# vmonardo/pnp-svrg

Measured on AMD Instinct MI355X. Metric: PnP-SVRG inner-iters/sec, 256x256 CSMRI+DnCNN, higher is better.
Workload: dtype f32; 1 GPU; pnp_svrg (true SVRG direction, T2=10, mb=1000) on 256x256 CSMRI, 20% Bernoulli mask, DnCNN-17 prox (reference DnCNN_noise15 weights); batch_per_gpu=120, problems_total=120, parallelism=replicas x1 (no data-path collective)

## Files before the change

### include/pnp_hip.h

```cpp
#ifndef PNP_HIP_H
#define PNP_HIP_H
#include <stddef.h>
#include <stdint.h>

#ifdef __cplusplus
extern "C" {
#endif

enum { PNP_F32 = 0, PNP_F64 = 1 };
enum { PNP_OK = 0, PNP_ERR_ARG = 1, PNP_ERR_HIP = 2, PNP_ERR_UNSUPPORTED = 3 };

int pnp_version(void);
const char* pnp_last_error(void);

typedef struct pnp_csmri_plan pnp_csmri_plan;

int pnp_csmri_plan_create(pnp_csmri_plan** plan, int H, int W, int batch, int dtype);
int pnp_csmri_plan_destroy(pnp_csmri_plan* plan);

int pnp_csmri_sel_from_indices(pnp_csmri_plan* plan, const int32_t* idx, int n, uint8_t* selT, void* stream);
int pnp_csmri_pack_mask(pnp_csmri_plan* plan, const uint8_t* selT, uint32_t* bitsT, void* stream);

int pnp_csmri_draw_thresholds(pnp_csmri_plan* plan, const uint32_t* bitsT, int mb, uint64_t seed, uint32_t step0,
                              int nsteps, const uint32_t* step_dev, void* mbd, uint32_t* selbits, void* stream);
// ... 62 lines not shown

int pnp_minmax(const void* z, int n_per_problem, int batch, int dtype, void* out, void* stream);

typedef struct pnp_dncnn_plan pnp_dncnn_plan;
int pnp_dncnn_plan_create(pnp_dncnn_plan** plan, int n_mid, const float* w_first, const float* w_mid,
                          const float* b_mid, const float* w_last, int H, int W, int batch);
int pnp_dncnn_plan_destroy(pnp_dncnn_plan* plan);
int pnp_dncnn_set_affine(pnp_dncnn_plan* plan, const float* b_first, float b_last, float negative_slope);
int pnp_dncnn_set_winograd(pnp_dncnn_plan* plan, int enable);
int pnp_dncnn_forward(pnp_dncnn_plan* plan, const float* x, float* r, void* stream);
int pnp_dncnn_denoise(pnp_dncnn_plan* plan, const void* z_in, void* z_out, int dtype, double sigma_net,
                      const void* xrec, double* sse_out, void* stream);

int pnp_mmo_denoise(pnp_dncnn_plan* plan, const void* z_in, void* z_out, int dtype, const void* xrec,
                    double* sse_out, void* stream);

int pnp_dncnn_profile_begin(pnp_dncnn_plan* plan, int max_calls);
int pnp_dncnn_profile_end(pnp_dncnn_plan* plan, double* avg_ms_per_launch, long* launches);
int pnp_dncnn_debug_clock(pnp_dncnn_plan* plan, int reps, double* cycles, double* ref_ticks, void* stream);
size_t pnp_dncnn_debug_w44_floats(void);
int pnp_dncnn_debug_w44_weights(pnp_dncnn_plan* plan, int layer, float* dst, void* stream);
int pnp_dncnn_debug_mid_layer(pnp_dncnn_plan* plan, int layer, const float* in, float* out, const float* w44_override,
                              int w44_rows, void* stream);

int pnp_counter_add(uint32_t* counter, uint32_t inc, void* stream);
int pnp_log_append(const double* src, int n, double* log, int n_log, const uint32_t* step_dev, void* stream);
int pnp_log_append_inc(const double* src, int n, double* log, int n_log, uint32_t* counter, void* stream);

int pnp_draw_thresholds(int M, int batch, int mb, uint64_t seed, uint32_t step0, int nsteps, const uint32_t* step_dev,
                        void* mbd, void* stream);
int pnp_indicator_from_thresholds(int M, int batch, const void* mbd, uint8_t* sel, void* stream);
int pnp_rows_from_thresholds(int M, int batch, int mb, const void* mbd, int32_t* rows, void* stream);
int pnp_indicator_from_indices(const int32_t* idx, int n, int M, int batch, uint8_t* sel, void* stream);
int pnp_saga_table_update(void* z, const void* g, void* slot, const void* prev, void* sum, double lr, double inv_hist,
                          size_t n, int dtype, void* stream);

int pnp_axpbypcz(double a, const void* x, double b, const void* y, double c, const void* w,
                 void* out, size_t n, int dtype, void* stream);

int pnp_legacy_choice(uint32_t* mt_key, int* mt_pos, const int64_t* pool, int pop, int size, int32_t* work, int64_t* out);

#ifdef __cplusplus
}
#endif
#endif
```

### pnp_svrg_amd/_native.py

```python
import ctypes
import os

_HERE = os.path.dirname(os.path.abspath(__file__))
LIB_PATH = os.environ.get('PNP_HIP_LIB') or os.path.join(_HERE, 'lib', 'libpnp_hip.so')

F32, F64 = 0, 1

_vp = ctypes.c_void_p
_i = ctypes.c_int
_d = ctypes.c_double
_sz = ctypes.c_size_t

SIGNATURES = {
    'pnp_version': (_i, []),
    'pnp_last_error': (ctypes.c_char_p, []),
    'pnp_csmri_plan_create': (_i, [ctypes.POINTER(_vp), _i, _i, _i, _i]),
    'pnp_csmri_plan_destroy': (_i, [_vp]),
    'pnp_csmri_sel_from_indices': (_i, [_vp, _vp, _i, _vp, _vp]),
    'pnp_csmri_pack_mask': (_i, [_vp, _vp, _vp, _vp]),
    'pnp_csmri_draw_thresholds': (_i, [_vp, _vp, _i, ctypes.c_uint64, ctypes.c_uint32, _i, _vp, _vp, _vp, _vp]),
    'pnp_csmri_sel_from_thresholds': (_i, [_vp, _vp, _vp, _vp, _vp]),
    'pnp_csmri_draw_minibatch': (_i, [_vp, _vp, _i, ctypes.c_uint64, ctypes.c_uint32, _vp, _vp, _vp]),
    'pnp_counter_add': (_i, [_vp, ctypes.c_uint32, _vp]),
    'pnp_log_append': (_i, [_vp, _i, _vp, _i, _vp, _vp]),
# ... 12 lines not shown
    'pnp_deblur_forward': (_i, [_vp, _vp, _vp, _vp]),
    'pnp_pr_workspace_elems': (_sz, [_i, _i]),
    'pnp_pr_grad': (_i, [_vp, _vp, _vp, _vp, _i, _i, _i, _i, _d, _vp, _vp, _vp]),
    'pnp_pr_grad_batch': (_i, [_vp, _vp, _vp, _vp, _i, _i, _i, _i, _i, _d, _vp, _vp, _vp]),
    'pnp_pr_spectral_apply': (_i, [_vp, _vp, _vp, _i, _i, _i, _d, _vp, _vp, _vp]),
    'pnp_sigma_est': (_i, [_vp, _i, _i, _i, _i, _vp, _vp]),
    'pnp_prox_tv': (_i, [_vp, _vp, _i, _i, _i, _i, _vp, _d, _d, _vp, _vp, _vp, _vp]),
    'pnp_nlm2d': (_i, [_vp, _vp, _i, _i, _i, _i, _i, _i, _vp, _d, _d, _vp, _d, _vp, _vp, _vp, _vp]),
    'pnp_sse': (_i, [_vp, _vp, _i, _i, _i, _vp, _vp]),
    'pnp_minmax': (_i, [_vp, _i, _i, _i, _vp, _vp]),
    'pnp_dncnn_plan_create': (_i, [ctypes.POINTER(_vp), _i, _vp, _vp, _vp, _vp, _i, _i, _i]),
    'pnp_dncnn_plan_destroy': (_i, [_vp]),
    'pnp_dncnn_set_affine': (_i, [_vp, _vp, ctypes.c_float, ctypes.c_float]),
    'pnp_dncnn_set_winograd': (_i, [_vp, _i]),
    'pnp_dncnn_forward': (_i, [_vp, _vp, _vp, _vp]),
    'pnp_dncnn_denoise': (_i, [_vp, _vp, _vp, _i, _d, _vp, _vp, _vp]),
    'pnp_mmo_denoise': (_i, [_vp, _vp, _vp, _i, _vp, _vp, _vp]),
    'pnp_dncnn_profile_begin': (_i, [_vp, _i]),
    'pnp_dncnn_profile_end': (_i, [_vp, ctypes.POINTER(_d), ctypes.POINTER(ctypes.c_long)]),
    'pnp_dncnn_debug_clock': (_i, [_vp, _i, ctypes.POINTER(_d), ctypes.POINTER(_d), _vp]),
    'pnp_dncnn_debug_w44_floats': (_sz, []),
    'pnp_dncnn_debug_w44_weights': (_i, [_vp, _i, _vp, _vp]),
    'pnp_dncnn_debug_mid_layer': (_i, [_vp, _i, _vp, _vp, _vp, _i, _vp]),
    'pnp_draw_thresholds': (_i, [_i, _i, _i, ctypes.c_uint64, ctypes.c_uint32, _i, _vp, _vp, _vp]),
    'pnp_indicator_from_thresholds': (_i, [_i, _i, _vp, _vp, _vp]),
    'pnp_rows_from_thresholds': (_i, [_i, _i, _i, _vp, _vp, _vp]),
    'pnp_indicator_from_indices': (_i, [_vp, _i, _i, _i, _vp, _vp]),
    'pnp_saga_table_update': (_i, [_vp, _vp, _vp, _vp, _vp, _d, _d, _sz, _i, _vp]),
    'pnp_axpbypcz': (_i, [_d, _vp, _d, _vp, _d, _vp, _vp, _sz, _i, _vp]),
    'pnp_legacy_choice': (_i, [_vp, ctypes.POINTER(ctypes.c_int), _vp, _i, _i, _vp, _vp]),
}

_lib = None


class NativeError(RuntimeError):
    pass


def lib():
    global _lib
    if _lib is None:
        if not os.path.exists(LIB_PATH):
            raise NativeError(
                f'{LIB_PATH} not found: build it with `python -c "import __graft_entry__ as g; g.build()"` '
                '(or `make -C pnp_svrg_amd/csrc`). There is no CPU fallback.')
# ... 18 lines not shown
```

### pnp_svrg_amd/csrc/dncnn.hip

```cpp
#include "common.h"
#include "wino44.h"
#include "wino44b.h"
#include "tilewalk.h"
#include "reduce.h"
#include <vector>
#include <algorithm>
#include <cstdlib>

namespace pnp {

using f32x4 = __attribute__((ext_vector_type(4))) float;

constexpr int C = 64;
constexpr int TR = 8, TC = 32;
constexpr int PR = TR + 2;
constexpr int PC = 40;
constexpr int XOFF = 3;
constexpr int PLANE = PR * PC;
constexpr int HALF_C = 32;
constexpr int HALF_PAYLOAD = HALF_C * PLANE;
constexpr int HALF_LDS = 52 * 256;
constexpr int CHUNKS = HALF_PAYLOAD / 4;
constexpr int KSTEPS_HALF = 9 * (HALF_C / 4);
constexpr int MT = 16;

__device__ __forceinline__ void dma_piece(int pc, const float* __restrict__ in, const float* __restrict__ zeros,
                                          float* ldsbuf, int H, int W, int b, int ty0, int tx0, int half, int lane,
                                          bool valid_tile) {
    const int q = pc * 64 + lane;
    const int cin = q / 100, r = q - cin * 100;
// ... 450 lines not shown
                const T lo = mm[2 * b], hi = mm[2 * b + 1];
                T v = (zin[p] - lo) / (hi - lo);
                v = v * (T)srange + (T)sshift;
                v = v - (T)r[j];
                v = (v - (T)sshift) / (T)srange;
                v = v * (hi - lo) + lo;
                zout[p] = v;
                if (xrec != nullptr) {
                    const double d = (double)xrec[p] - (double)v;
                    err += d * d;
                }
            }
        }
    }
    if (sse_part != nullptr) {
        err = wave_sum(err);
        if ((tid & 63) == 0) red[tid >> 6] = err;
        __syncthreads();
        if (tid == 0)
            sse_part[((size_t)b * gridDim.y + blockIdx.y) * gridDim.x + blockIdx.x] = red[0] + red[1] + red[2] + red[3];
    }
}

__global__ void k_sum_parts(const double* __restrict__ part, int nparts, double* __restrict__ out) {
    double s = 0;
    for (int i = threadIdx.x; i < nparts; i += 64) s += part[(size_t)blockIdx.x * nparts + i];
    s = wave_sum(s);
    if (threadIdx.x == 0) out[blockIdx.x] = s;
}

}

using namespace pnp;

struct pnp_dncnn_plan {
    int n_mid, H, W, batch, num_cu;
    float *w_first, *w_last, *wpack, *upack, *bias;
    float* upack44;
    uint16_t* upack44b;
    float* b_first;
    float b_last, slope;
    int use_wino;
    float *act0, *act1, *zeros;
    double* mm;
    double* sse_part;
    bool profile;
    std::vector<hipEvent_t> ev;
    size_t ev_used;
    double prof_ms;
    long prof_launches;
};

extern "C" int pnp_dncnn_plan_create(pnp_dncnn_plan** out, int n_mid, const float* w_first, const float* w_mid,
                                     const float* b_mid, const float* w_last, int H, int W, int batch) {
    PNP_CHECK_ARG(out && w_first && w_mid && b_mid && w_last, "null argument");
    PNP_CHECK_ARG(n_mid >= 1 && batch >= 1, "n_mid and batch must be >= 1");
    PNP_CHECK_ARG(H % TR == 0 && W % TC == 0 && (H * W) % 256 == 0, "H must be a multiple of 8, W of 32");
    auto* p = new pnp_dncnn_plan{};
    p->n_mid = n_mid; p->H = H; p->W = W; p->batch = batch;
    hipDeviceProp_t prop;
    int dev = 0;
    PNP_CHECK_HIP(hipGetDevice(&dev));
    PNP_CHECK_HIP(hipGetDeviceProperties(&prop, dev));
    p->num_cu = prop.multiProcessorCount;
    std::vector<float> pack((size_t)n_mid * 4 * 2 * KSTEPS_HALF * 64);
// ... 3 lines not shown
                for (int lane = 0; lane < 64; ++lane) {
                    const int half = s / KSTEPS_HALF, rs = s % KSTEPS_HALF, tap = rs / (HALF_C / 4), c4 = rs % (HALF_C / 4);
                    const int cout = 16 * wv + (lane & 15), cin = HALF_C * half + 4 * c4 + (lane >> 4);
                    pack[(((size_t)l * 4 + wv) * 2 * KSTEPS_HALF + s) * 64 + lane] =
                        w_mid[(((size_t)l * C + cout) * C + cin) * 9 + tap];
                }
    std::vector<float> upk((size_t)n_mid * 4 * WINO_U * 64);
    for (int l = 0; l < n_mid; ++l)
        for (int wv = 0; wv < 4; ++wv)
            for (int s = 0; s < WINO_U; ++s)
                for (int lane = 0; lane < 64; ++lane) {
                    const int xi = s % 4, dy = (s / 4) % 3, c4 = (s / 12) % (HALF_C / 4), half = s / (12 * (HALF_C / 4));
                    const int cout = 16 * wv + (lane & 15), cin = HALF_C * half + 4 * c4 + (lane >> 4);
                    const float* g = w_mid + (((size_t)l * C + cout) * C + cin) * 9 + dy * 3;
                    const double g0 = g[0], g1 = g[1], g2 = g[2];
                    const double u = xi == 0 ? g0 : xi == 1 ? 0.5 * (g0 + g1 + g2) : xi == 2 ? 0.5 * (g0 - g1 + g2) : g2;
                    upk[(((size_t)l * 4 + wv) * WINO_U + s) * 64 + lane] = (float)u;
                }
    {
        const char* ev = getenv("PNP_DNCNN_WINOGRAD");
        p->use_wino = ev ? atoi(ev) : 5;
        if (p->use_wino != 6 && p->use_wino != 5 && p->use_wino != 1 && p->use_wino != 0) p->use_wino = 5;
        if (p->use_wino >= 5 && !wino44_supports(H, W)) p->use_wino = 1;
    }
    const size_t act_bytes = (size_t)batch * C * H * W * sizeof(float);
    hipError_t e = hipMalloc(&p->wpack, pack.size() * sizeof(float));
    if (e == hipSuccess) e = hipMemcpy(p->wpack, pack.data(), pack.size() * sizeof(float), hipMemcpyHostToDevice);
    if (e == hipSuccess) e = hipMalloc(&p->upack, upk.size() * sizeof(float));
    if (e == hipSuccess) e = hipMemcpy(p->upack, upk.data(), upk.size() * sizeof(float), hipMemcpyHostToDevice);
    {
        std::vector<float> u44(wino44_weight_floats(n_mid));
        wino44_pack_weights(w_mid, n_mid, u44.data());
        if (e == hipSuccess) e = hipMalloc(&p->upack44, u44.size() * sizeof(float));
        if (e == hipSuccess) e = hipMemcpy(p->upack44, u44.data(), u44.size() * sizeof(float), hipMemcpyHostToDevice);
    }
    if (wino44b_supports(H, W)) {
        std::vector<uint16_t> u44b(wino44b_weight_halfwords(n_mid));
        wino44b_pack_weights(w_mid, n_mid, u44b.data());
        if (e == hipSuccess) e = hipMalloc(&p->upack44b, u44b.size() * sizeof(uint16_t));
        if (e == hipSuccess) e = hipMemcpy(p->upack44b, u44b.data(), u44b.size() * sizeof(uint16_t), hipMemcpyHostToDevice);
    }
    if (e == hipSuccess) e = hipMalloc(&p->bias, (size_t)n_mid * C * sizeof(float));
    if (e == hipSuccess) e = hipMemcpy(p->bias, b_mid, (size_t)n_mid * C * sizeof(float), hipMemcpyHostToDevice);
    if (e == hipSuccess) e = hipMalloc(&p->w_first, C * 9 * sizeof(float));
    if (e == hipSuccess) e = hipMemcpy(p->w_first, w_first, C * 9 * sizeof(float), hipMemcpyHostToDevice);
    if (e == hipSuccess) e = hipMalloc(&p->w_last, C * 9 * sizeof(float));
    if (e == hipSuccess) e = hipMemcpy(p->w_last, w_last, C * 9 * sizeof(float), hipMemcpyHostToDevice);
    if (e == hipSuccess) e = hipMalloc(&p->b_first, C * sizeof(float));
    if (e == hipSuccess) e = hipMemset(p->b_first, 0, C * sizeof(float));
    if (e == hipSuccess) e = hipMalloc(&p->act0, act_bytes);
    if (e == hipSuccess) e = hipMalloc(&p->act1, act_bytes);
    if (e == hipSuccess) e = hipMalloc(&p->zeros, 256);
    if (e == hipSuccess) e = hipMemset(p->zeros, 0, 256);
    if (e == hipSuccess) e = hipMalloc(&p->mm, (size_t)batch * 2 * sizeof(double));
    if (e == hipSuccess) e = hipMalloc(&p->sse_part, (size_t)batch * (H * W / 256) * sizeof(double));
    if (e != hipSuccess) {
        set_error(std::string("pnp_dncnn_plan_create: ") + hipGetErrorString(e));
        for (void* q : {(void*)p->wpack, (void*)p->upack, (void*)p->bias, (void*)p->w_first, (void*)p->w_last, (void*)p->act0,
                        (void*)p->act1, (void*)p->zeros, (void*)p->mm, (void*)p->sse_part, (void*)p->b_first, (void*)p->upack44,
                        (void*)p->upack44b})
            if (q) (void)hipFree(q);
        delete p;
        return PNP_ERR_HIP;
    }
    *out = p;
    return PNP_OK;
}

extern "C" int pnp_dncnn_plan_destroy(pnp_dncnn_plan* p) {
    if (!p) return PNP_OK;
    for (void* q : {(void*)p->wpack, (void*)p->upack, (void*)p->bias, (void*)p->w_first, (void*)p->w_last, (void*)p->act0, (void*)p->act1,
                    (void*)p->zeros, (void*)p->mm, (void*)p->sse_part, (void*)p->b_first, (void*)p->upack44, (void*)p->upack44b})
        (void)hipFree(q);
    for (hipEvent_t e : p->ev) (void)hipEventDestroy(e);
    delete p;
    return PNP_OK;
}

namespace {
template <typename T>
int run_dncnn(pnp_dncnn_plan* p, const T* z_in, bool normalise, double sigma_net, T* z_out, float* r_out,
              const T* xrec, double* sse_out, hipStream_t s, bool mmo = false) {
    const int H = p->H, W = p->W, B = p->batch, HW = H * W;
    T* mm = normalise ? (T*)p->mm : nullptr;
    double srange = 1.0, sshift = 0.0;
    if (normalise) {
        k_minmax<T><<<B, 256, 0, s>>>(z_in, HW, mm);
        PNP_CHECK_LAUNCH();
        srange = 1.0 + sigma_net / 255.0 / 2.0;
        sshift = (1.0 - srange) / 2.0;
    }
    dim3 pg(HW / 256, B);
    k_first<T><<<pg, 256, 0, s>>>(z_in, mm, p->w_first, p->b_first, p->act0, H, W, srange, sshift, mmo ? 1 : 0, p->slope);
    PNP_CHECK_LAUNCH();
    const int ntiles = B * (H / TR) * (W / TC);
    const int grid = ntiles < p->num_cu ? ntiles : p->num_cu;
    float *src = p->act0, *dst = p->act1;
    const bool prof = p->profile && p->ev_used + 2 <= p->ev.size();
    if (prof) PNP_CHECK_HIP(hipEventRecord(p->ev[p->ev_used], s));
    for (int l = 0; l < p->n_mid; ++l) {
        if (p->use_wino == 6) {
            const int rc = wino44b_layer(src, dst, p->upack44b + (size_t)l * wino44b_weight_halfwords(1), p->bias + (size_t)l * C,
                                         H, W, B, p->num_cu, p->slope, s);
            if (rc != PNP_OK) return rc;
        } else if (p->use_wino == 5) {
            const int rc = wino44_layer(src, dst, p->upack44 + (size_t)l * wino44_weight_floats(1), p->bias + (size_t)l * C, p->zeros,
                                        H, W, B, p->num_cu, p->slope, s);
            if (rc != PNP_OK) return rc;
        } else if (p->slope != 0.f) {
            if (p->use_wino)
                k_mid_wino<true, false, true><<<grid, 256, 0, s>>>(src, dst, p->upack + (size_t)l * 4 * WINO_U * 64,
                                                                  p->bias + (size_t)l * C, p->zeros, H, W, ntiles, nullptr, p->slope);
            else
                k_mid<true, false, 0, true><<<grid, 256, 0, s>>>(src, dst, p->wpack + (size_t)l * 4 * 2 * KSTEPS_HALF * 64,
                                                                p->bias + (size_t)l * C, p->zeros, H, W, ntiles, nullptr, p->slope);
        } else if (p->use_wino)
            k_mid_wino<true><<<grid, 256, 0, s>>>(src, dst, p->upack + (size_t)l * 4 * WINO_U * 64, p->bias + (size_t)l * C,
                                                  p->zeros, H, W, ntiles);
        else
            k_mid<true><<<grid, 256, 0, s>>>(src, dst, p->wpack + (size_t)l * 4 * 2 * KSTEPS_HALF * 64, p->bias + (size_t)l * C,
                                             p->zeros, H, W, ntiles);
        PNP_CHECK_LAUNCH();
        float* t = src; src = dst; dst = t;
    }
    if (prof) { PNP_CHECK_HIP(hipEventRecord(p->ev[p->ev_used + 1], s)); p->ev_used += 2; }
    dim3 lg((W + LT_C - 1) / LT_C, (H + LT_R - 1) / LT_R, B);
    k_last<T><<<lg, 256, 0, s>>>(src, p->w_last, z_in, mm, z_out, r_out, xrec, sse_out ? p->sse_part : nullptr, H, W,
                                 srange, sshift, mmo ? 1 : 0, p->b_last);
    PNP_CHECK_LAUNCH();
    if (sse_out) {
        k_sum_parts<<<B, 64, 0, s>>>(p->sse_part, (int)(lg.x * lg.y), sse_out);
        PNP_CHECK_LAUNCH();
    }
    return PNP_OK;
}
}

extern "C" size_t pnp_dncnn_debug_w44_floats(void) { return wino44_weight_floats(1); }

extern "C" int pnp_dncnn_debug_w44_weights(pnp_dncnn_plan* p, int layer, float* dst, void* stream) {
    PNP_CHECK_ARG(p && dst && layer >= 0 && layer < p->n_mid, "bad argument");
    PNP_CHECK_HIP(hipMemcpyAsync(dst, p->upack44 + (size_t)layer * wino44_weight_floats(1), wino44_weight_floats(1) * sizeof(float),
                                 hipMemcpyDeviceToDevice, (hipStream_t)stream));
    return PNP_OK;
}

extern "C" int pnp_dncnn_debug_mid_layer(pnp_dncnn_plan* p, int layer, const float* in, float* out, const float* w44_override,
                                         int w44_rows, void* stream) {
    PNP_CHECK_ARG(p && in && out && layer >= 0 && layer < p->n_mid && w44_rows >= 0 && w44_rows <= 2, "bad argument");
    PNP_CHECK_ARG(w44_override == nullptr || p->use_wino == 5, "w44_override needs the F(4x4,3x3) kernel (mode 5)");
    hipStream_t s = (hipStream_t)stream;
    const int H = p->H, W = p->W, B = p->batch, l = layer;
    const int ntiles = B * (H / TR) * (W / TC);
    const int grid = ntiles < p->num_cu ? ntiles : p->num_cu;
    if (p->use_wino == 6)
        return wino44b_layer(in, out, p->upack44b + (size_t)l * wino44b_weight_halfwords(1), p->bias + (size_t)l * C, H, W, B, p->num_cu,
                             p->slope, s);
    if (p->use_wino == 5)
        return wino44_layer(in, out, w44_override ? w44_override : p->upack44 + (size_t)l * wino44_weight_floats(1),
                            p->bias + (size_t)l * C, p->zeros, H, W, B, p->num_cu, p->slope, s, w44_rows);
    PNP_CHECK_ARG(p->slope == 0.f, "the hook runs the ReLU builds of the direct / F(2,3) kernels");
    if (p->use_wino)
        k_mid_wino<true><<<grid, 256, 0, s>>>(in, out, p->upack + (size_t)l * 4 * WINO_U * 64, p->bias + (size_t)l * C, p->zeros, H, W, ntiles);
    else
        k_mid<true><<<grid, 256, 0, s>>>(in, out, p->wpack + (size_t)l * 4 * 2 * KSTEPS_HALF * 64, p->bias + (size_t)l * C, p->zeros, H, W, ntiles);
    PNP_CHECK_LAUNCH();
    return PNP_OK;
}

extern "C" int pnp_dncnn_set_affine(pnp_dncnn_plan* p, const float* b_first, float b_last, float negative_slope) {
    PNP_CHECK_ARG(p != nullptr, "null plan");
    PNP_CHECK_ARG(negative_slope >= 0.f && negative_slope < 1.f, "negative_slope must be in [0, 1)");
    if (b_first) PNP_CHECK_HIP(hipMemcpy(p->b_first, b_first, C * sizeof(float), hipMemcpyHostToDevice));
    else PNP_CHECK_HIP(hipMemset(p->b_first, 0, C * sizeof(float)));
    p->b_last = b_last;
    p->slope = negative_slope;
    return PNP_OK;
}

extern "C" int pnp_dncnn_set_winograd(pnp_dncnn_plan* p, int enable) {
    PNP_CHECK_ARG(p != nullptr, "null plan");
    PNP_CHECK_ARG(enable == 0 || enable == 1 || enable == 5 || enable == 6,
                  "mode must be 0 (direct), 1 (Winograd F(2,3) along x), 5 (Winograd F(4x4,3x3)) or 6 (the same on 3 x bf16 splits)");
    PNP_CHECK_ARG(!(enable >= 5 && !wino44_supports(p->H, p->W)), "Winograd F(4x4,3x3) needs H % 8 == 0 and W % 64 == 0");
    p->use_wino = enable;
    return PNP_OK;
}

extern "C" int pnp_dncnn_profile_begin(pnp_dncnn_plan* p, int max_calls) {
    PNP_CHECK_ARG(p && max_calls > 0, "bad argument");
// ... 116 lines not shown
```

### pnp_svrg_amd/csrc/dncnn_wino44.hip

```cpp
#include "common.h"
#include "wino44.h"
#include "tilewalk.h"
#include <vector>
#include <utility>
#include <cstdlib>

namespace pnp {
namespace w44 {

using f32x4 = __attribute__((ext_vector_type(4))) float;
using f32x2 = __attribute__((ext_vector_type(2))) float;

constexpr int C = 64;
constexpr int TC = 64;
constexpr int PC = 72;
constexpr int KC = 8;
constexpr int NCH = C / KC;
template <int NG_> struct Geo {
    static constexpr int NG = NG_;
    static constexpr int TR = 4 * NG, PR = TR + 2;
    static constexpr int PLANE = NG == 2 ? 768 : 512;
    static constexpr int DBUF = KC * PLANE;
    static constexpr int PPW = DBUF / 256 / 4;
    static constexpr int VPL = 128 * NG;
// ... 201 lines not shown
    __syncthreads();
    if (STAMP) t_wait += __builtin_amdgcn_s_memtime() - ta;
}
template <bool STAMP, int VAR, typename CT, typename MK, int... K> __device__ __forceinline__ void all_chunks(CT& c, MK&& mk, unsigned long long& t_wait, std::integer_sequence<int, K...>) {
    (chunk<K, STAMP, VAR>(c, mk(std::integral_constant<int, K>{}), t_wait), ...);
}

template <int VPL> __device__ __forceinline__ void transform0(const float* dsrc, float* vdst) {
    float t[6][6];
#pragma unroll
    for (int r = 0; r < 6; ++r) {
        const float* row = dsrc + r * PC;
        bt6(row[3], row[4], row[5], row[6], row[7], row[8], t[r]);
    }
#pragma unroll
    for (int x = 0; x < 6; ++x) {
        float v[6];
        bt6(t[0][x], t[1][x], t[2][x], t[3][x], t[4][x], t[5][x], v);
#pragma unroll
        for (int y = 0; y < 6; ++y) vdst[(y * 6 + x) * VPL] = v[y];
    }
}

template <bool LEAKY, int NG = 2, bool STAMP = false, int VAR = 0>
__global__ __launch_bounds__(256, 1) void k_mid_wino44(const float* __restrict__ in, float* __restrict__ out,
                                                       const float4* __restrict__ upack, const float* __restrict__ bias,
                                                       int H, int W, int ntiles, float slope,
                                                       unsigned long long* __restrict__ stamps = nullptr, int tile0 = 0) {
    using G = Geo<NG>;
    constexpr int TR = G::TR, PR = G::PR, PLANE = G::PLANE, DBUF = G::DBUF, PPW = G::PPW, VPL = G::VPL, VBUF = G::VBUF;
    __shared__ __attribute__((aligned(16))) float lds[G::LDS_FLOATS];
    const int tid = threadIdx.x, lane = tid & 63, wv = __builtin_amdgcn_readfirstlane(tid >> 6);
    const int tiles_x = W / TC, units_per_img = tiles_x * (H / 8);
    auto region = [&](int u, int& b, int& ty0, int& tx0) {
        const int t = tile0 + (NG == 2 ? u : u >> 1);
        b = t / units_per_img;
        const int t2 = t - b * units_per_img;
        ty0 = (t2 / tiles_x) * 8 + (NG == 2 ? 0 : 4 * (u & 1));
        tx0 = (t2 % tiles_x) * TC;
    };

    float bv[4];
#pragma unroll
    for (int r = 0; r < 4; ++r) bv[r] = bias[16 * wv + 4 * (lane >> 4) + r];

    const int tc = lane & 15, j = (lane >> 4) & 1, g = NG == 2 ? lane >> 5 : 0;
    const int d_off = 4 * ((2 * wv + j) * (PLANE / 4) + g * PC + tc);
    const ptrdiff_t hw4 = (ptrdiff_t)4 * H * W, w4 = (ptrdiff_t)4 * W;
    const unsigned st_off = 4u * (unsigned)(4 * (lane >> 4) * H * W + 4 * tc);
    const int v_off = g * 128 + wv * 32 + tc * 2 + j;

    unsigned pdesc[PPW];
#pragma unroll
    for (int i = 0; i < PPW; ++i) {
// ... 24 lines not shown
        return rs;
    };
    auto dma_piece = [&](const TileDma& td, i32x4 rs, int buf, int i) {
        dma_piece_asm(td.voff[i], rs, lds0 + 4u * (unsigned)(buf * DBUF + (wv + 4 * i) * 256));
    };

    float* const dbuf = lds;
    float* const vbuf = lds + 2 * DBUF;

    Ctx<NG> c;
    lds_f* const ldsp = (lds_f*)lds;
    c.dsrc[0] = ldsp + d_off;                     c.dsrc[1] = ldsp + DBUF + d_off;
    c.vdst[0] = ldsp + 2 * DBUF + v_off;          c.vdst[1] = ldsp + 2 * DBUF + VBUF + v_off;
    c.vsrc0[0] = ldsp + 2 * DBUF + 2 * lane;      c.vsrc0[1] = ldsp + 2 * DBUF + VBUF + 2 * lane;
    c.vsrc1[0] = c.vsrc0[0] + 128;                c.vsrc1[1] = c.vsrc0[1] + 128;
    asm volatile("" : "+v"(c.vsrc1[0]), "+v"(c.vsrc1[1]));
    const __attribute__((address_space(1))) char* const ubase = (const __attribute__((address_space(1))) char*)upack + (size_t)(wv * NCH * 18) * 1024;
    c.ucur = ubase;
    c.ulane = 16u * lane;

    const TileWalk tw_ = tile_walk(ntiles);
    int tile = tw_.first;
    const int limit = tw_.limit < ntiles ? tw_.limit : ntiles;
    {
        const TileDma td0 = tile_dma(tile < limit ? tile : ntiles);
#pragma unroll
        for (int i = 0; i < PPW; ++i) dma_piece(td0, chunk_rsrc(td0, 0), 0, i);
#pragma unroll
        for (int i = 0; i < PPW; ++i) dma_piece(td0, chunk_rsrc(td0, 1), 1, i);
#pragma unroll
        for (int i = 0; i < URING; ++i) c.ur[i] = c.uload_next();
        asm volatile("s_waitcnt vmcnt(0)" ::: "memory");
        __syncthreads();
        transform0<VPL>(dbuf + d_off, vbuf + v_off);
        __syncthreads();
    }

    unsigned long long t0 = 0, r0 = 0, t_wait = 0, t_epi = 0;
    if (STAMP) { t0 = __builtin_amdgcn_s_memtime(); r0 = __builtin_amdgcn_s_memrealtime(); }
    for (; tile < limit; tile += tw_.step) {
        asm volatile("" : "+v"(c.ulane));
        int b, ty0, tx0;
        region(tile, b, ty0, tx0);
        const int ntile = tile + tw_.step < limit ? tile + tw_.step : ntiles;

        const TileDma cur = tile_dma(tile), nxt = tile_dma(ntile);
        all_chunks<STAMP, VAR>(c, [&](auto kc) {
            constexpr int K = decltype(kc)::value;
            const TileDma& td = K + 2 < NCH ? cur : nxt;
            const i32x4 rs = chunk_rsrc(td, (K + 2) % NCH);
            return [&, rs](int piece) { dma_piece(td, rs, K & 1, piece); };
        }, t_wait, std::make_integer_sequence<int, NCH>{});

        unsigned long long te = 0;
        if (STAMP) te = __builtin_amdgcn_s_memtime();
        asm volatile("; W44_EPILOGUE_BEGIN\n\ts_nop 15\n\ts_nop 7" ::: "memory");
#pragma unroll
        for (int g2 = 0; g2 < NG; ++g2)
#pragma unroll
            for (int xi = 0; xi < 36; xi += 4) {
                if (G::in_agpr(g2, xi)) asm volatile("" : "+a"(c.acc[g2][xi]), "+a"(c.acc[g2][xi + 1]), "+a"(c.acc[g2][xi + 2]), "+a"(c.acc[g2][xi + 3]));
                else asm volatile("" : "+v"(c.acc[g2][xi]), "+v"(c.acc[g2][xi + 1]), "+v"(c.acc[g2][xi + 2]), "+v"(c.acc[g2][xi + 3]));
            }
        unsigned so = st_off;
        asm volatile("" : "+v"(so));
        __attribute__((address_space(1))) char* const ob = (__attribute__((address_space(1))) char*)out + 4 * ((((size_t)b * C + 16 * wv) * H + ty0) * (size_t)W + tx0);
#pragma unroll
        for (int blk = 0; blk < 2 * NG; ++blk) {
            {
                const int g2 = NG == 2 ? 1 - (blk >> 1) : 0, pi = blk & 1;
                if (blk == 2 * NG - 1) {
                    c.ucur = ubase;
#pragma unroll
                    for (int i = 0; i < URING; ++i) c.ur[i] = c.uload_next();
                    __builtin_amdgcn_sched_barrier(0);
                }
                const f32x2 bias2 = {bv[2 * pi], bv[2 * pi + 1]};
                __attribute__((address_space(1))) char* oc = ob + (ptrdiff_t)(2 * pi) * hw4 + (ptrdiff_t)(4 * g2) * w4;
                asm volatile("" : "+s"(oc));
                f32x2 s[6][4];
#pragma unroll
                for (int x = 0; x < 6; ++x) {
                    f32x2 m[6];
#pragma unroll
                    for (int y = 0; y < 6; ++y) {
                        const f32x4 q = c.acc[g2][6 * y + x];
                        m[y] = pi ? f32x2{q.z, q.w} : f32x2{q.x, q.y};
                    }
                    if (x == 1) m[1] += bias2;
                    at6(m[0], m[1], m[2], m[3], m[4], m[5], s[x]);
                    if (x & 1) __builtin_amdgcn_sched_barrier(0);
                }
#pragma unroll
                for (int r = 0; r < 4; ++r) {
                    f32x2 y[4];
                    at6(s[0][r], s[1][r], s[2][r], s[3][r], s[4][r], s[5][r], y);
                    f32x4 v0, v1;
                    if (LEAKY) {
                        v0.x = fmaxf(y[0].x, slope * y[0].x); v0.y = fmaxf(y[1].x, slope * y[1].x);
                        v0.z = fmaxf(y[2].x, slope * y[2].x); v0.w = fmaxf(y[3].x, slope * y[3].x);
                        v1.x = fmaxf(y[0].y, slope * y[0].y); v1.y = fmaxf(y[1].y, slope * y[1].y);
                        v1.z = fmaxf(y[2].y, slope * y[2].y); v1.w = fmaxf(y[3].y, slope * y[3].y);
                    } else {
                        v0.x = fmaxf(y[0].x, 0.f); v0.y = fmaxf(y[1].x, 0.f); v0.z = fmaxf(y[2].x, 0.f); v0.w = fmaxf(y[3].x, 0.f);
                        v1.x = fmaxf(y[0].y, 0.f); v1.y = fmaxf(y[1].y, 0.f); v1.z = fmaxf(y[2].y, 0.f); v1.w = fmaxf(y[3].y, 0.f);
                    }
                    *(__attribute__((address_space(1))) f32x4*)(oc + so) = v0;
                    oc += hw4;
                    asm volatile("" : "+s"(oc));
                    *(__attribute__((address_space(1))) f32x4*)(oc + so) = v1;
                    oc += w4 - hw4;
                    asm volatile("" : "+s"(oc));
                    if (r & 1) __builtin_amdgcn_sched_barrier(0);
                }
            }
        }
        asm volatile("; W44_EPILOGUE_END" ::: "memory");
        if (STAMP) t_epi += __builtin_amdgcn_s_memtime() - te;
    }
    if (STAMP && tid == 0) {
        stamps[4 * blockIdx.x] = __builtin_amdgcn_s_memtime() - t0;
        stamps[4 * blockIdx.x + 1] = __builtin_amdgcn_s_memrealtime() - r0;
        stamps[4 * blockIdx.x + 2] = t_wait;
        stamps[4 * blockIdx.x + 3] = t_epi;
    }
}

}

bool wino44_supports(int H, int W) { return H % 8 == 0 && W % w44::TC == 0; }

size_t wino44_weight_floats(int n_mid) { return (size_t)n_mid * 4 * w44::NCH * 18 * 64 * 4; }

void wino44_pack_weights(const float* w_mid, int n_mid, float* out) {
    static const double G[6][3] = {{1.0 / 4, 0, 0}, {-1.0 / 6, -1.0 / 6, -1.0 / 6}, {-1.0 / 6, 1.0 / 6, -1.0 / 6},
                                   {1.0 / 24, 1.0 / 12, 1.0 / 6}, {1.0 / 24, -1.0 / 12, 1.0 / 6}, {0, 0, 1}};
    for (int l = 0; l < n_mid; ++l)
        for (int wv = 0; wv < 4; ++wv)
            for (int k = 0; k < w44::NCH; ++k)
                for (int lane = 0; lane < 64; ++lane)
                    for (int j = 0; j < 2; ++j) {
                        const int cout = 16 * wv + (lane & 15), cin = w44::KC * k + 2 * (lane >> 4) + j;
                        const float* g = w_mid + (((size_t)l * w44::C + cout) * w44::C + cin) * 9;
                        for (int xy = 0; xy < 6; ++xy)
                            for (int xx = 0; xx < 6; ++xx) {
                                double u = 0;
                                for (int dy = 0; dy < 3; ++dy)
                                    for (int dx = 0; dx < 3; ++dx) u += G[xy][dy] * G[xx][dx] * (double)g[dy * 3 + dx];
                                const int xi = 6 * xy + xx, p = xi >> 1, e = 2 * (xi & 1) + j;
                                out[((((size_t)(l * 4 + wv) * w44::NCH + k) * 18 + p) * 64 + lane) * 4 + e] = (float)u;
                            }
                    }
}

int wino44_layer(const float* in, float* out, const float* upack_layer, const float* bias, const float* zeros, int H, int W,
                 int batch, int num_cu, float slope, hipStream_t s, int force) {
    const int units = batch * (H / 8) * (W / w44::TC);
    int full = force == 1 ? 0 : force == 2 ? units : (units / num_cu) * num_cu;
    if (force == 0 && 2 * (units - full) > num_cu) full = units;
    const float4* up = (const float4*)upack_layer;
    if (full > 0) {
        const int grid = full < num_cu ? full : num_cu;
        if (slope != 0.f) w44::k_mid_wino44<true, 2><<<grid, 256, 0, s>>>(in, out, up, bias, H, W, full, slope, nullptr, 0);
        else w44::k_mid_wino44<false, 2><<<grid, 256, 0, s>>>(in, out, up, bias, H, W, full, 0.f, nullptr, 0);
        PNP_CHECK_LAUNCH();
    }
    if (full < units) {
        const int n1 = 2 * (units - full), grid = n1 < num_cu ? n1 : num_cu;
        if (slope != 0.f) w44::k_mid_wino44<true, 1><<<grid, 256, 0, s>>>(in, out, up, bias, H, W, n1, slope, nullptr, full);
        else w44::k_mid_wino44<false, 1><<<grid, 256, 0, s>>>(in, out, up, bias, H, W, n1, 0.f, nullptr, full);
        PNP_CHECK_LAUNCH();
    }
    return PNP_OK;
}

int wino44_debug_clock(const float* in, float* out, const float* upack_layer, const float* bias, int H, int W, int batch,
                       int num_cu, int reps, unsigned long long* stamps_dev, hipStream_t s) {
    const int ntiles = batch * (H / 8) * (W / w44::TC);
    const int grid = ntiles < num_cu ? ntiles : num_cu;
    for (int i = 0; i < reps - 1; ++i)
        w44::k_mid_wino44<false, 2><<<grid, 256, 0, s>>>(in, out, (const float4*)upack_layer, bias, H, W, ntiles, 0.f);
    const int var = getenv("PNP_W44_VAR") ? atoi(getenv("PNP_W44_VAR")) : 0;
    if (var == 0) w44::k_mid_wino44<false, 2, true><<<grid, 256, 0, s>>>(in, out, (const float4*)upack_layer, bias, H, W, ntiles, 0.f, stamps_dev);
#ifdef PNP_W44_ABLATIONS
#define PNP_W44_ABL(V) else if (var == V) w44::k_mid_wino44<false, 2, true, V><<<grid, 256, 0, s>>>(in, out, (const float4*)upack_layer, bias, H, W, ntiles, 0.f, stamps_dev);
    PNP_W44_ABL(10) PNP_W44_ABL(11) PNP_W44_ABL(12) PNP_W44_ABL(13) PNP_W44_ABL(14) PNP_W44_ABL(15)
#undef PNP_W44_ABL
#endif
    else PNP_CHECK_ARG(false, "PNP_W44_VAR: this library was built without -DPNP_W44_ABLATIONS");
    PNP_CHECK_LAUNCH();
    return PNP_OK;
}
// ... 3 lines not shown
```

### pnp_svrg_amd/csrc/wino44.h

```cpp
#pragma once
#include "common.h"

namespace pnp {
bool wino44_supports(int H, int W);
size_t wino44_weight_floats(int n_mid);
void wino44_pack_weights(const float* w_mid, int n_mid, float* out);
int wino44_layer(const float* in, float* out, const float* upack_layer, const float* bias, const float* zeros, int H, int W,
                 int batch, int num_cu, float slope, hipStream_t s, int force_rows = 0);
int wino44_debug_clock(const float* in, float* out, const float* upack_layer, const float* bias, int H, int W, int batch,
                       int num_cu, int reps, unsigned long long* stamps_dev, hipStream_t s);
}
```

### pnp_svrg_amd/ops.py

```python
import ctypes
import torch
from . import _native as N

_DT = {torch.float32: N.F32, torch.float64: N.F64}
_CDT = {torch.float32: torch.complex64, torch.float64: torch.complex128}


def _stream():
    try:
        return ctypes.c_void_p(torch._C._cuda_getCurrentRawStream(torch._C._cuda_getDevice()))
    except AttributeError:
        return ctypes.c_void_p(torch.cuda.current_stream().cuda_stream)


def _p(t):
    if t is None:
        return None
    assert t.is_cuda and t.is_contiguous(), 'device-resident contiguous tensors only'
    return ctypes.c_void_p(t.data_ptr())


def require_gpu():
    if not torch.cuda.is_available():
        raise N.NativeError('no MI355X visible (torch.cuda.is_available() is False); the hot path has no CPU fallback')
# ... 159 lines not shown
                N.lib().pnp_dncnn_plan_destroy(h)
            except Exception:
                pass

    def profile_begin(self, max_calls=4096):
        N.call('pnp_dncnn_profile_begin', self._h, int(max_calls))

    def profile_end(self):
        ms, n = ctypes.c_double(), ctypes.c_long()
        N.call('pnp_dncnn_profile_end', self._h, ctypes.byref(ms), ctypes.byref(n))
        return ms.value, n.value

    def debug_w44_weights(self, layer):
        n = N.lib().pnp_dncnn_debug_w44_floats()
        dst = torch.empty(n, dtype=torch.float32, device='cuda')
        N.call('pnp_dncnn_debug_w44_weights', self._h, int(layer), _p(dst), _stream())
        return dst

    def debug_mid_layer(self, layer, x, out, w44=None, rows=0):
        assert x.dtype == torch.float32 and tuple(x.shape) == (self.B, 64, self.H, self.W) and tuple(out.shape) == tuple(x.shape)
        N.call('pnp_dncnn_debug_mid_layer', self._h, int(layer), _p(x), _p(out), _p(w44), int(rows), _stream())
        return out

    def forward(self, x, out=None):
        assert x.dtype == torch.float32 and tuple(x.shape) == (self.B, self.H, self.W)
        out = out if out is not None else torch.empty_like(x)
        N.call('pnp_dncnn_forward', self._h, _p(x), _p(out), _stream())
        return out

    def denoise(self, z, sigma_net, xrec=None, out=None, sse=None):
        assert tuple(z.shape) == (self.B, self.H, self.W)
        out = out if out is not None else torch.empty_like(z)
        if xrec is not None and sse is None:
            sse = torch.empty(self.B, dtype=torch.float64, device=z.device)
        N.call('pnp_dncnn_denoise', self._h, _p(z), _p(out), _DT[z.dtype], float(sigma_net), _p(xrec), _p(sse), _stream())
        return out, sse


    def mmo_denoise(self, z, xrec=None, out=None, sse=None):
        assert tuple(z.shape) == (self.B, self.H, self.W)
        out = out if out is not None else torch.empty_like(z)
        if xrec is not None and sse is None:
            sse = torch.empty(self.B, dtype=torch.float64, device=z.device)
        N.call('pnp_mmo_denoise', self._h, _p(z), _p(out), _DT[z.dtype], _p(xrec), _p(sse), _stream())
        return out, sse

# ... 209 lines not shown
```

Measured before the change: 5165 inner-iters/s.

## Fuse DnCNN last conv into final Winograd mid layer via per-tile partial patches

Result: faster. 5261 inner-iters/s, median of 6 (+1.9%).

```diff
diff --git a/include/pnp_hip.h b/include/pnp_hip.h
--- a/include/pnp_hip.h
+++ b/include/pnp_hip.h
@@ -108,6 +108,7 @@
 int pnp_dncnn_debug_w44_weights(pnp_dncnn_plan* plan, int layer, float* dst, void* stream);
 int pnp_dncnn_debug_mid_layer(pnp_dncnn_plan* plan, int layer, const float* in, float* out, const float* w44_override,
                               int w44_rows, void* stream);
+int pnp_dncnn_debug_fused_last(pnp_dncnn_plan* plan, const float* in, float* part, int w44_rows, void* stream);
 
 int pnp_counter_add(uint32_t* counter, uint32_t inc, void* stream);
 int pnp_log_append(const double* src, int n, double* log, int n_log, const uint32_t* step_dev, void* stream);
diff --git a/pnp_svrg_amd/_native.py b/pnp_svrg_amd/_native.py
--- a/pnp_svrg_amd/_native.py
+++ b/pnp_svrg_amd/_native.py
@@ -58,6 +58,7 @@
     'pnp_dncnn_debug_w44_floats': (_sz, []),
     'pnp_dncnn_debug_w44_weights': (_i, [_vp, _i, _vp, _vp]),
     'pnp_dncnn_debug_mid_layer': (_i, [_vp, _i, _vp, _vp, _vp, _i, _vp]),
+    'pnp_dncnn_debug_fused_last': (_i, [_vp, _vp, _vp, _i, _vp]),
     'pnp_draw_thresholds': (_i, [_i, _i, _i, ctypes.c_uint64, ctypes.c_uint32, _i, _vp, _vp, _vp]),
     'pnp_indicator_from_thresholds': (_i, [_i, _i, _vp, _vp, _vp]),
     'pnp_rows_from_thresholds': (_i, [_i, _i, _i, _vp, _vp, _vp]),
diff --git a/pnp_svrg_amd/csrc/dncnn.hip b/pnp_svrg_amd/csrc/dncnn.hip
--- a/pnp_svrg_amd/csrc/dncnn.hip
+++ b/pnp_svrg_amd/csrc/dncnn.hip
@@ -6,6 +6,7 @@
 #include <vector>
 #include <algorithm>
 #include <cstdlib>
+#include <type_traits>
 
 namespace pnp {
 
@@ -502,6 +503,51 @@
     }
 }
 
+template <typename T>
+__global__ __launch_bounds__(256) void k_last_patches(const float* __restrict__ part, const T* zin, const T* __restrict__ mm,
+                                                      T* zout, float* __restrict__ r_out, const T* __restrict__ xrec,
+                                                      double* __restrict__ sse_part, int H, int W, double srange, double sshift,
+                                                      float blast) {
+    __shared__ double red[4];
+    const int tid = threadIdx.x, b = blockIdx.z;
+    const int iy = tid >> 6, ix = tid & 3, bx = blockIdx.x * 16 + ((tid >> 2) & 15), by = blockIdx.y;
+    const int y = 4 * by + iy, x = 4 * bx + ix;
+    const int NBX = W / 4, NBY = H / 4;
+    const float* pb = part + (size_t)b * NBY * NBX * 36;
+    auto at = [&](int qy, int qx, int py, int px) { return pb[((size_t)qy * NBX + qx) * 36 + py * 6 + px]; };
+    const int vy = iy == 0 ? -1 : iy == 3 ? 1 : 0, vx = ix == 0 ? -1 : ix == 3 ? 1 : 0;
+    const bool hv = vy != 0 && by + vy >= 0 && by + vy < NBY, hh = vx != 0 && bx + vx >= 0 && bx + vx < NBX;
+    const int py = iy + 1, px = ix + 1, pyn = py - 4 * vy, pxn = px - 4 * vx;
+    float r = at(by, bx, py, px);
+    if (hv) r += at(by + vy, bx, pyn, px);
+    if (hh) r += at(by, bx + vx, py, pxn);
+    if (hv && hh) r += at(by + vy, bx + vx, pyn, pxn);
+    r += blast;
+    const size_t p = (size_t)b * H * W + (size_t)y * W + x;
+    if (r_out != nullptr) r_out[p] = r;
+    double err = 0.0;
+    if (zout != nullptr) {
+        const T lo = mm ? mm[2 * b] : (T)0, hi = mm ? mm[2 * b + 1] : (T)1;
+        T v = (zin[p] - lo) / (hi - lo);
+        v = v * (T)srange + (T)sshift;
+        v = v - (T)r;
+        v = (v - (T)sshift) / (T)srange;
+        v = v * (hi - lo) + lo;
+        zout[p] = v;
+        if (xrec != nullptr) {
+            const double d = (double)xrec[p] - (double)v;
+            err = d * d;
+        }
+    }
+    if (sse_part != nullptr) {
+        err = wave_sum(err);
+        if ((tid & 63) == 0) red[tid >> 6] = err;
+        __syncthreads();
+        if (tid == 0)
+            sse_part[((size_t)b * gridDim.y + blockIdx.y) * gridDim.x + blockIdx.x] = red[0] + red[1] + red[2] + red[3];
+    }
+}
+
 __global__ void k_sum_parts(const double* __restrict__ part, int nparts, double* __restrict__ out) {
     double s = 0;
     for (int i = threadIdx.x; i < nparts; i += 64) s += part[(size_t)blockIdx.x * nparts + i];
@@ -521,6 +567,8 @@
     float* b_first;
     float b_last, slope;
     int use_wino;
+    bool edge_fusion;
+    float* part;
     float *act0, *act1, *zeros;
     double* mm;
     double* sse_part;
@@ -570,6 +618,8 @@
         p->use_wino = ev ? atoi(ev) : 5;
         if (p->use_wino != 6 && p->use_wino != 5 && p->use_wino != 1 && p->use_wino != 0) p->use_wino = 5;
         if (p->use_wino >= 5 && !wino44_supports(H, W)) p->use_wino = 1;
+        const char* ef = getenv("PNP_DNCNN_EDGE_FUSION");
+        p->edge_fusion = !(ef && atoi(ef) == 0);
     }
     const size_t act_bytes = (size_t)batch * C * H * W * sizeof(float);
     hipError_t e = hipMalloc(&p->wpack, pack.size() * sizeof(float));
@@ -602,11 +652,12 @@
     if (e == hipSuccess) e = hipMemset(p->zeros, 0, 256);
     if (e == hipSuccess) e = hipMalloc(&p->mm, (size_t)batch * 2 * sizeof(double));
     if (e == hipSuccess) e = hipMalloc(&p->sse_part, (size_t)batch * (H * W / 256) * sizeof(double));
+    if (e == hipSuccess && wino44_supports(H, W)) e = hipMalloc(&p->part, wino44_part_floats(H, W, batch) * sizeof(float));
     if (e != hipSuccess) {
         set_error(std::string("pnp_dncnn_plan_create: ") + hipGetErrorString(e));
         for (void* q : {(void*)p->wpack, (void*)p->upack, (void*)p->bias, (void*)p->w_first, (void*)p->w_last, (void*)p->act0,
                         (void*)p->act1, (void*)p->zeros, (void*)p->mm, (void*)p->sse_part, (void*)p->b_first, (void*)p->upack44,
-                        (void*)p->upack44b})
+                        (void*)p->upack44b, (void*)p->part})
             if (q) (void)hipFree(q);
         delete p;
         return PNP_ERR_HIP;
@@ -618,7 +669,8 @@
 extern "C" int pnp_dncnn_plan_destroy(pnp_dncnn_plan* p) {
     if (!p) return PNP_OK;
     for (void* q : {(void*)p->wpack, (void*)p->upack, (void*)p->bias, (void*)p->w_first, (void*)p->w_last, (void*)p->act0, (void*)p->act1,
-                    (void*)p->zeros, (void*)p->mm, (void*)p->sse_part, (void*)p->b_first, (void*)p->upack44, (void*)p->upack44b})
+                    (void*)p->zeros, (void*)p->mm, (void*)p->sse_part, (void*)p->b_first, (void*)p->upack44, (void*)p->upack44b,
+                    (void*)p->part})
         (void)hipFree(q);
     for (hipEvent_t e : p->ev) (void)hipEventDestroy(e);
     delete p;
@@ -644,6 +696,8 @@
     const int ntiles = B * (H / TR) * (W / TC);
     const int grid = ntiles < p->num_cu ? ntiles : p->num_cu;
     float *src = p->act0, *dst = p->act1;
+    const bool fuse_last = p->edge_fusion && p->use_wino == 5 && p->slope == 0.f && !mmo && std::is_same<T, float>::value &&
+                           p->part != nullptr;
     const bool prof = p->profile && p->ev_used + 2 <= p->ev.size();
     if (prof) PNP_CHECK_HIP(hipEventRecord(p->ev[p->ev_used], s));
     for (int l = 0; l < p->n_mid; ++l) {
@@ -652,8 +706,9 @@
                                          H, W, B, p->num_cu, p->slope, s);
             if (rc != PNP_OK) return rc;
         } else if (p->use_wino == 5) {
+            const bool fl = fuse_last && l == p->n_mid - 1;
             const int rc = wino44_layer(src, dst, p->upack44 + (size_t)l * wino44_weight_floats(1), p->bias + (size_t)l * C, p->zeros,
-                                        H, W, B, p->num_cu, p->slope, s);
+                                        H, W, B, p->num_cu, p->slope, s, 0, fl ? p->w_last : nullptr, fl ? p->part : nullptr);
             if (rc != PNP_OK) return rc;
         } else if (p->slope != 0.f) {
             if (p->use_wino)
@@ -672,6 +727,17 @@
         float* t = src; src = dst; dst = t;
     }
     if (prof) { PNP_CHECK_HIP(hipEventRecord(p->ev[p->ev_used + 1], s)); p->ev_used += 2; }
+    if (fuse_last) {
+        const dim3 fg(W / 64, H / 4, B);
+        k_last_patches<T><<<fg, 256, 0, s>>>(p->part, z_in, mm, z_out, r_out, xrec, sse_out ? p->sse_part : nullptr, H, W, srange,
+                                             sshift, p->b_last);
+        PNP_CHECK_LAUNCH();
+        if (sse_out) {
+            k_sum_parts<<<B, 64, 0, s>>>(p->sse_part, (int)(fg.x * fg.y), sse_out);
+            PNP_CHECK_LAUNCH();
+        }
+        return PNP_OK;
+    }
     dim3 lg((W + LT_C - 1) / LT_C, (H + LT_R - 1) / LT_R, B);
     k_last<T><<<lg, 256, 0, s>>>(src, p->w_last, z_in, mm, z_out, r_out, xrec, sse_out ? p->sse_part : nullptr, H, W,
                                  srange, sshift, mmo ? 1 : 0, p->b_last);
@@ -714,6 +780,15 @@
         k_mid<true><<<grid, 256, 0, s>>>(in, out, p->wpack + (size_t)l * 4 * 2 * KSTEPS_HALF * 64, p->bias + (size_t)l * C, p->zeros, H, W, ntiles);
     PNP_CHECK_LAUNCH();
     return PNP_OK;
+}
+
+extern "C" int pnp_dncnn_debug_fused_last(pnp_dncnn_plan* p, const float* in, float* part, int w44_rows, void* stream) {
+    PNP_CHECK_ARG(p && in && part && w44_rows >= 0 && w44_rows <= 2, "bad argument");
+    PNP_CHECK_ARG(p->use_wino == 5 && p->slope == 0.f && p->part != nullptr,
+                  "the fused last layer needs the F(4x4,3x3) kernel (mode 5) and ReLU");
+    const int l = p->n_mid - 1;
+    return wino44_layer(in, nullptr, p->upack44 + (size_t)l * wino44_weight_floats(1), p->bias + (size_t)l * C, p->zeros, p->H, p->W,
+                        p->batch, p->num_cu, 0.f, (hipStream_t)stream, w44_rows, p->w_last, part);
 }
 
 extern "C" int pnp_dncnn_set_affine(pnp_dncnn_plan* p, const float* b_first, float b_last, float negative_slope) {
diff --git a/pnp_svrg_amd/csrc/dncnn_wino44.hip b/pnp_svrg_amd/csrc/dncnn_wino44.hip
--- a/pnp_svrg_amd/csrc/dncnn_wino44.hip
+++ b/pnp_svrg_amd/csrc/dncnn_wino44.hip
@@ -247,14 +247,20 @@
     }
 }
 
-template <bool LEAKY, int NG = 2, bool STAMP = false, int VAR = 0>
+constexpr int FL_PATCH = 36;
+constexpr int FL_BLK = 16 * FL_PATCH;
+template <int NG, bool FL> constexpr int fl_lds_floats() { return FL ? C * 9 + NG * 4 * FL_BLK : 0; }
+
+template <bool LEAKY, int NG = 2, bool STAMP = false, int VAR = 0, bool FL = false>
 __global__ __launch_bounds__(256, 1) void k_mid_wino44(const float* __restrict__ in, float* __restrict__ out,
                                                        const float4* __restrict__ upack, const float* __restrict__ bias,
                                                        int H, int W, int ntiles, float slope,
-                                                       unsigned long long* __restrict__ stamps = nullptr, int tile0 = 0) {
+                                                       unsigned long long* __restrict__ stamps = nullptr, int tile0 = 0,
+                                                       const float* __restrict__ wlast = nullptr, float* __restrict__ part = nullptr) {
     using G = Geo<NG>;
     constexpr int TR = G::TR, PR = G::PR, PLANE = G::PLANE, DBUF = G::DBUF, PPW = G::PPW, VPL = G::VPL, VBUF = G::VBUF;
-    __shared__ __attribute__((aligned(16))) float lds[G::LDS_FLOATS];
+    static_assert(!(FL && LEAKY), "the fused last layer is built for the ReLU net");
+    __shared__ __attribute__((aligned(16))) float lds[G::LDS_FLOATS + fl_lds_floats<NG, FL>()];
     const int tid = threadIdx.x, lane = tid & 63, wv = __builtin_amdgcn_readfirstlane(tid >> 6);
     const int tiles_x = W / TC, units_per_img = tiles_x * (H / 8);
     auto region = [&](int u, int& b, int& ty0, int& tx0) {
@@ -325,6 +331,10 @@
     const TileWalk tw_ = tile_walk(ntiles);
     int tile = tw_.first;
     const int limit = tw_.limit < ntiles ? tw_.limit : ntiles;
+    float* const flw = lds + G::LDS_FLOATS;
+    float* const flx = flw + C * 9;
+    if constexpr (FL)
+        for (int i = tid; i < C * 9; i += 256) flw[i] = wlast[i];
     {
         const TileDma td0 = tile_dma(tile < limit ? tile : ntiles);
 #pragma unroll
@@ -368,10 +378,20 @@
         unsigned so = st_off;
         asm volatile("" : "+v"(so));
         __attribute__((address_space(1))) char* const ob = (__attribute__((address_space(1))) char*)out + 4 * ((((size_t)b * C + 16 * wv) * H + ty0) * (size_t)W + tx0);
+        float q[FL_PATCH];
 #pragma unroll
         for (int blk = 0; blk < 2 * NG; ++blk) {
             {
                 const int g2 = NG == 2 ? 1 - (blk >> 1) : 0, pi = blk & 1;
+                float wr[2][9];
+                if constexpr (FL) {
+                    if (pi == 0)
+#pragma unroll
+                        for (int i = 0; i < FL_PATCH; ++i) q[i] = 0.f;
+                    const float* wc = flw + (16 * wv + 4 * (lane >> 4) + 2 * pi) * 9;
+#pragma unroll
+                    for (int t = 0; t < 9; ++t) { wr[0][t] = wc[t]; wr[1][t] = wc[9 + t]; }
+                }
                 if (blk == 2 * NG - 1) {
                     c.ucur = ubase;
 #pragma unroll
@@ -408,14 +428,56 @@
                         v0.x = fmaxf(y[0].x, 0.f); v0.y = fmaxf(y[1].x, 0.f); v0.z = fmaxf(y[2].x, 0.f); v0.w = fmaxf(y[3].x, 0.f);
                         v1.x = fmaxf(y[0].y, 0.f); v1.y = fmaxf(y[1].y, 0.f); v1.z = fmaxf(y[2].y, 0.f); v1.w = fmaxf(y[3].y, 0.f);
                     }
-                    *(__attribute__((address_space(1))) f32x4*)(oc + so) = v0;
-                    oc += hw4;
-                    asm volatile("" : "+s"(oc));
-                    *(__attribute__((address_space(1))) f32x4*)(oc + so) = v1;
-                    oc += w4 - hw4;
-                    asm volatile("" : "+s"(oc));
+                    if constexpr (FL) {
+                        const float a0[4] = {v0.x, v0.y, v0.z, v0.w}, a1[4] = {v1.x, v1.y, v1.z, v1.w};
+#pragma unroll
+                        for (int dy = 0; dy < 3; ++dy)
+#pragma unroll
+                            for (int dx = 0; dx < 3; ++dx)
+#pragma unroll
+                                for (int k = 0; k < 4; ++k) {
+                                    float& d = q[(r + 2 - dy) * 6 + k + 2 - dx];
+                                    d = __builtin_fmaf(wr[0][dy * 3 + dx], a0[k], d);
+                                    d = __builtin_fmaf(wr[1][dy * 3 + dx], a1[k], d);
+                                }
+                    } else {
+                        *(__attribute__((address_space(1))) f32x4*)(oc + so) = v0;
+                        oc += hw4;
+                        asm volatile("" : "+s"(oc));
+                        *(__attribute__((address_space(1))) f32x4*)(oc + so) = v1;
+                        oc += w4 - hw4;
+                        asm volatile("" : "+s"(oc));
+                    }
                     if (r & 1) __builtin_amdgcn_sched_barrier(0);
                 }
+                if constexpr (FL) {
+                    if (pi == 1) {
+                        const bool h32 = (lane & 32) != 0, h16 = (lane & 16) != 0;
+                        float k1[18], k2[9];
+#pragma unroll
+                        for (int i = 0; i < 18; ++i) {
+                            const float mine = h32 ? q[18 + i] : q[i], give = h32 ? q[i] : q[18 + i];
+                            k1[i] = mine + __shfl_xor(give, 32);
+                        }
+#pragma unroll
+                        for (int i = 0; i < 9; ++i) {
+                            const float mine = h16 ? k1[9 + i] : k1[i], give = h16 ? k1[i] : k1[9 + i];
+                            k2[i] = mine + __shfl_xor(give, 16);
+                        }
+                        float* const xd = flx + (g2 * 4 + wv) * FL_BLK + tc * FL_PATCH + 9 * (lane >> 4);
+#pragma unroll
+                        for (int i = 0; i < 9; ++i) xd[i] = k2[i];
+                    }
+                }
+            }
+        }
+        if constexpr (FL) {
+            __syncthreads();
+            float* const pb = part + (((size_t)b * (H / 4) + ty0 / 4) * (size_t)(W / 4) + tx0 / 4) * FL_PATCH;
+            for (int e = tid; e < NG * FL_BLK; e += 256) {
+                const int g2 = e >= FL_BLK ? 1 : 0, rem = e - g2 * FL_BLK;
+                const float* xs = flx + g2 * 4 * FL_BLK + rem;
+                pb[(size_t)g2 * (W / 4) * FL_PATCH + rem] = ((xs[0] + xs[FL_BLK]) + xs[2 * FL_BLK]) + xs[3 * FL_BLK];
             }
         }
         asm volatile("; W44_EPILOGUE_END" ::: "memory");
@@ -457,20 +519,23 @@
 }
 
 int wino44_layer(const float* in, float* out, const float* upack_layer, const float* bias, const float* zeros, int H, int W,
-                 int batch, int num_cu, float slope, hipStream_t s, int force) {
+                 int batch, int num_cu, float slope, hipStream_t s, int force, const float* wlast, float* part) {
+    PNP_CHECK_ARG(part == nullptr || (slope == 0.f && wlast != nullptr), "the fused last layer needs ReLU and w_last");
     const int units = batch * (H / 8) * (W / w44::TC);
     int full = force == 1 ? 0 : force == 2 ? units : (units / num_cu) * num_cu;
     if (force == 0 && 2 * (units - full) > num_cu) full = units;
     const float4* up = (const float4*)upack_layer;
     if (full > 0) {
         const int grid = full < num_cu ? full : num_cu;
-        if (slope != 0.f) w44::k_mid_wino44<true, 2><<<grid, 256, 0, s>>>(in, out, up, bias, H, W, full, slope, nullptr, 0);
+        if (part) w44::k_mid_wino44<false, 2, false, 0, true><<<grid, 256, 0, s>>>(in, out, up, bias, H, W, full, 0.f, nullptr, 0, wlast, part);
+        else if (slope != 0.f) w44::k_mid_wino44<true, 2><<<grid, 256, 0, s>>>(in, out, up, bias, H, W, full, slope, nullptr, 0);
         else w44::k_mid_wino44<false, 2><<<grid, 256, 0, s>>>(in, out, up, bias, H, W, full, 0.f, nullptr, 0);
         PNP_CHECK_LAUNCH();
     }
     if (full < units) {
         const int n1 = 2 * (units - full), grid = n1 < num_cu ? n1 : num_cu;
-        if (slope != 0.f) w44::k_mid_wino44<true, 1><<<grid, 256, 0, s>>>(in, out, up, bias, H, W, n1, slope, nullptr, full);
+        if (part) w44::k_mid_wino44<false, 1, false, 0, true><<<grid, 256, 0, s>>>(in, out, up, bias, H, W, n1, 0.f, nullptr, full, wlast, part);
+        else if (slope != 0.f) w44::k_mid_wino44<true, 1><<<grid, 256, 0, s>>>(in, out, up, bias, H, W, n1, slope, nullptr, full);
         else w44::k_mid_wino44<false, 1><<<grid, 256, 0, s>>>(in, out, up, bias, H, W, n1, 0.f, nullptr, full);
         PNP_CHECK_LAUNCH();
     }
diff --git a/pnp_svrg_amd/csrc/wino44.h b/pnp_svrg_amd/csrc/wino44.h
--- a/pnp_svrg_amd/csrc/wino44.h
+++ b/pnp_svrg_amd/csrc/wino44.h
@@ -6,7 +6,9 @@
 size_t wino44_weight_floats(int n_mid);
 void wino44_pack_weights(const float* w_mid, int n_mid, float* out);
 int wino44_layer(const float* in, float* out, const float* upack_layer, const float* bias, const float* zeros, int H, int W,
-                 int batch, int num_cu, float slope, hipStream_t s, int force_rows = 0);
+                 int batch, int num_cu, float slope, hipStream_t s, int force_rows = 0, const float* wlast = nullptr,
+                 float* part = nullptr);
+inline size_t wino44_part_floats(int H, int W, int batch) { return (size_t)batch * (H / 4) * (W / 4) * 36; }
 int wino44_debug_clock(const float* in, float* out, const float* upack_layer, const float* bias, int H, int W, int batch,
                        int num_cu, int reps, unsigned long long* stamps_dev, hipStream_t s);
 }
diff --git a/pnp_svrg_amd/ops.py b/pnp_svrg_amd/ops.py
--- a/pnp_svrg_amd/ops.py
+++ b/pnp_svrg_amd/ops.py
@@ -205,6 +205,12 @@
         N.call('pnp_dncnn_debug_mid_layer', self._h, int(layer), _p(x), _p(out), _p(w44), int(rows), _stream())
         return out
 
+    def debug_fused_last(self, x, part, rows=0):
+        assert x.dtype == torch.float32 and tuple(x.shape) == (self.B, 64, self.H, self.W)
+        assert part.dtype == torch.float32 and part.numel() == self.B * (self.H // 4) * (self.W // 4) * 36
+        N.call('pnp_dncnn_debug_fused_last', self._h, _p(x), _p(part), int(rows), _stream())
+        return part
+
     def forward(self, x, out=None):
         assert x.dtype == torch.float32 and tuple(x.shape) == (self.B, self.H, self.W)
         out = out if out is not None else torch.empty_like(x)
```
